# m1el/nemotron-asr.cpp

Hardware: AMD Instinct MI355X
Metric: RTFx (audio-sec/sec), nemotron-0.6B streaming forward path (higher is better)
Workload: dtype bf16

## Files before the change

nemotron-asr.cpp_amd/csrc/kernels_fused.hip:

```cpp
#include "nasr_internal.h"
#include "nasr_epilogue.h"
#include "nasr_wave.h"

namespace nasr {

typedef __attribute__((ext_vector_type(8))) __bf16 bf16x8;
typedef __attribute__((ext_vector_type(2))) __bf16 bf16x2;
typedef __attribute__((ext_vector_type(4))) float f32x4;
typedef __attribute__((ext_vector_type(4))) unsigned int u32x4;

__device__ __forceinline__ float wsum_f(float v) { return wave_sum(v); }
__device__ __forceinline__ float wmax_f(float v) { return wave_max(v); }

__device__ __forceinline__ int panel_byte(int row, int k, int KP) {
    const int chunk = k >> 3;
    return row * KP * 2 + (((chunk ^ (row & 15)) << 4) | ((k & 7) << 1));
}

__device__ __forceinline__ void store4_panel(char *panel, int row, int k, int KP, float a, float b, float c, float d) {
    uint2 r;
    r.x = (uint32_t)f32_to_bf16(a) | ((uint32_t)f32_to_bf16(b) << 16);
    r.y = (uint32_t)f32_to_bf16(c) | ((uint32_t)f32_to_bf16(d) << 16);
    *(uint2 *)(panel + panel_byte(row, k, KP)) = r;
}
// ... 1 lines not shown
__device__ __forceinline__ void wave_ln(float4 v[4], const float *w, const float *b, int lane) {
    float s = 0.f;
#pragma unroll
    for (int i = 0; i < 4; i++) s += (v[i].x + v[i].y) + (v[i].z + v[i].w);
    const float mean = wsum_f(s) * (1.0f / D);
    float q = 0.f;
#pragma unroll
    for (int i = 0; i < 4; i++) {
        v[i].x -= mean; v[i].y -= mean; v[i].z -= mean; v[i].w -= mean;
        q += (v[i].x * v[i].x + v[i].y * v[i].y) + (v[i].z * v[i].z + v[i].w * v[i].w);
    }
    const float inv = 1.0f / sqrtf(wsum_f(q) * (1.0f / D) + 1e-5f);
#pragma unroll
    for (int i = 0; i < 4; i++) {
        const int e = lane * 4 + 256 * i;
        const float4 ww = *(const float4 *)(w + e), bb = *(const float4 *)(b + e);
        v[i] = make_float4(v[i].x * inv * ww.x + bb.x, v[i].y * inv * ww.y + bb.y, v[i].z * inv * ww.z + bb.z, v[i].w * inv * ww.w + bb.w);
    }
}

__device__ __forceinline__ float bsum(float v, float *sh) {
    v = wsum_f(v);
    if ((threadIdx.x & 63) == 0) sh[threadIdx.x >> 6] = v;
    __syncthreads();
    return (sh[0] + sh[1]) + (sh[2] + sh[3]);
}
__device__ __forceinline__ float4 block_ln(float4 v, float4 ww, float4 bb, float *sh) {
    const float mean = bsum((v.x + v.y) + (v.z + v.w), sh) * (1.0f / D);
    const float dx = v.x - mean, dy = v.y - mean, dz = v.z - mean, dw = v.w - mean;
    const float var = bsum((dx * dx + dy * dy) + (dz * dz + dw * dw), sh + 4) * (1.0f / D);
    const float inv = 1.0f / sqrtf(var + 1e-5f);
    return make_float4(dx * inv * ww.x + bb.x, dy * inv * ww.y + bb.y, dz * inv * ww.z + bb.z, dw * inv * ww.w + bb.w);
}

template <bool BF16>
__device__ __forceinline__ float dot32(const float *qs, const void *row) {
    float s = 0.0f;
    if (BF16) {
        const uint4 *r = (const uint4 *)row;
#pragma unroll
        for (int c = 0; c < 4; c++) {
            const uint4 u = r[c];
            const uint32_t w[4] = {u.x, u.y, u.z, u.w};
#pragma unroll
            for (int e = 0; e < 4; e++) {
                s += qs[c * 8 + 2 * e] * __uint_as_float(w[e] << 16);
                s += qs[c * 8 + 2 * e + 1] * __uint_as_float(w[e] & 0xffff0000u);
            }
        }
    }
    return s;
}

#ifdef NASR_STAMPS
#define STAMP(i)                                                                                                         \
    do {                                                                                                                 \
        if (p.stamps && threadIdx.x == 0 && blockIdx.y == 0 && (blockIdx.x == 0 || blockIdx.x == gridDim.x - 1))          \
            p.stamps[(blockIdx.x == 0 ? 0 : 16) + (i)] = __builtin_amdgcn_s_memrealtime();                                \
    } while (0)
#else
#define STAMP(i)
#endif

#define PIN_SGPR(x) asm volatile("" ::"s"(x))

#ifndef GRP_OCC
#define GRP_OCC 4
#endif
template <int PRO, int MMAX>
__device__ __forceinline__ void fused_skinny_body(const FusedParams &p) {
    extern __shared__ __attribute__((aligned(16))) char smem[];
    const GemmParams &g = p.g;
    const int nt = blockIdx.x, split = blockIdx.y;
    const int wave = threadIdx.x >> 6, lane = threadIdx.x & 63;
    const int q = lane >> 4, r = lane & 15;
    const int KT = g.K >> 5;
    const int t0 = (int)((long)KT * split / g.splits), t1 = (int)((long)KT * (split + 1) / g.splits);
    const int KP = (t1 - t0) * 32;
    float *red = (float *)smem;
    char *panel = smem + 4096;
    const bool writer = blockIdx.x == 0 && blockIdx.y == 0;
    const int M = MMAX == 1 ? 1 : g.M;
    constexpr bool SMALL = MMAX <= 2;
    constexpr int MR = MMAX == 1 ? 1 : 2;
    STAMP(0);

    constexpr int U = (PRO == PRO_DWCONV && MMAX == 1) ? 2 : 8;
    const int nts = t1 - t0;
    const int w0 = t0 + nts * wave / 4, w1 = t0 + nts * (wave + 1) / 4;
    const u32x4 *wp = (const u32x4 *)g.W + (size_t)nt * KT * 64 + lane;
    u32x4 wv[U];
    auto issue_weights = [&]() {
        if (PRO == PRO_ATTN) {
#pragma unroll
            for (int u = 0; u < U; u++) {
                const int ntile = blockIdx.x * 8 + wave * 2 + (u >> 2), kt = t0 + (u & 3);
                wv[u] = __builtin_nontemporal_load((const u32x4 *)g.W + ((size_t)ntile * KT + kt) * 64 + lane);
            }
        } else {
#pragma unroll
            for (int u = 0; u < U; u++) {
                const int kt = w0 + u < w1 ? w0 + u : w1 - 1;
                wv[u] = __builtin_nontemporal_load(wp + (size_t)kt * 64);
            }
        }
        PIN_SGPR(g.epi); PIN_SGPR(g.out_f32); PIN_SGPR(g.ldo); PIN_SGPR(g.out_act); PIN_SGPR(g.ldo_act); PIN_SGPR(g.N);
        PIN_SGPR(g.q_out); PIN_SGPR(g.kv_pool); PIN_SGPR(g.kv_slot_stride); PIN_SGPR(g.rows); PIN_SGPR(g.T);
    };
    if (!((PRO == PRO_LN && SMALL) || PRO == PRO_ATTN || PRO == PRO_PLAIN || (PRO == PRO_DWCONV && SMALL))) issue_weights();
    STAMP(1);

    if (PRO == PRO_LN && SMALL) {
        const int c4 = threadIdx.x * 4;
        const float4 lw = *(const float4 *)(p.ln_w + c4), lb = *(const float4 *)(p.ln_b + c4);
        float4 ow = make_float4(0.f, 0.f, 0.f, 0.f), ob = ow;
        if (p.lno_w) { ow = *(const float4 *)(p.lno_w + c4); ob = *(const float4 *)(p.lno_b + c4); }
        float4 xv[MR], t[MR][8];
#pragma unroll
        for (int m = 0; m < MR; m++) {
            if (m < M) {
                xv[m] = *(const float4 *)(p.x_in + (size_t)m * D + c4);
#pragma unroll
                for (int sI = 0; sI < 8; sI++)
                    t[m][sI] = sI < p.part_splits ? *(const float4 *)(p.part + ((size_t)sI * M + m) * D + c4) : make_float4(0.f, 0.f, 0.f, 0.f);
            }
        }
        issue_weights();
#pragma unroll
        for (int m = 0; m < MR; m++) {
            if (m < M) {
                float4 v = xv[m];
                if (p.part_splits > 0) {
                    float4 o = t[m][0];
#pragma unroll
                    for (int sI = 1; sI < 8; sI++)
                        if (sI < p.part_splits) { o.x += t[m][sI].x; o.y += t[m][sI].y; o.z += t[m][sI].z; o.w += t[m][sI].w; }
                    v.x += p.scale * o.x; v.y += p.scale * o.y; v.z += p.scale * o.z; v.w += p.scale * o.w;
                }
                STAMP(2);
                if (p.lno_w) v = block_ln(v, ow, ob, red);
                if (writer && p.x_out) *(float4 *)(p.x_out + (size_t)m * D + c4) = v;
                v = block_ln(v, lw, lb, red);
                STAMP(3);
                store4_panel(panel, m, c4, KP, v.x, v.y, v.z, v.w);
            }
        }
        __syncthreads();
    } else if (PRO == PRO_LN) {
        float *xs = (float *)(panel + 16 * KP * 2);
        const int c4 = threadIdx.x * 4;
        for (int m0 = 0; m0 < M; m0 += 4) {
            float4 xv[4], t[4][8];
#pragma unroll
            for (int u = 0; u < 4; u++) {
                const int m = m0 + u < M ? m0 + u : M - 1;
                xv[u] = *(const float4 *)(p.x_in + (size_t)m * D + c4);
#pragma unroll
                for (int sI = 0; sI < 8; sI++)
                    t[u][sI] = sI < p.part_splits ? *(const float4 *)(p.part + ((size_t)sI * M + m) * D + c4) : make_float4(0.f, 0.f, 0.f, 0.f);
            }
#pragma unroll
            for (int u = 0; u < 4; u++) {
                const int m = m0 + u;
                if (m < M) {
                    float4 v = xv[u];
                    if (p.part_splits > 0) {
                        float4 o = t[u][0];
#pragma unroll
                        for (int sI = 1; sI < 8; sI++)
                            if (sI < p.part_splits) { o.x += t[u][sI].x; o.y += t[u][sI].y; o.z += t[u][sI].z; o.w += t[u][sI].w; }
                        v.x += p.scale * o.x; v.y += p.scale * o.y; v.z += p.scale * o.z; v.w += p.scale * o.w;
                    }
                    *(float4 *)(xs + (size_t)m * D + c4) = v;
                    if (writer && p.x_out && !p.lno_w) *(float4 *)(p.x_out + (size_t)m * D + c4) = v;
                }
            }
        }
        __syncthreads();
        for (int m = wave; m < M; m += 4) {
            float4 v[4];
#pragma unroll
            for (int i = 0; i < 4; i++) v[i] = *(const float4 *)(xs + (size_t)m * D + lane * 4 + 256 * i);
            if (p.lno_w) {
                wave_ln(v, p.lno_w, p.lno_b, lane);
                if (writer && p.x_out) {
#pragma unroll
                    for (int i = 0; i < 4; i++) *(float4 *)(p.x_out + (size_t)m * D + lane * 4 + 256 * i) = v[i];
                }
            }
            wave_ln(v, p.ln_w, p.ln_b, lane);
#pragma unroll
            for (int i = 0; i < 4; i++) store4_panel(panel, m, lane * 4 + 256 * i, KP, v[i].x, v[i].y, v[i].z, v[i].w);
        }
        __syncthreads();
    } else if (PRO == PRO_ATTN) {
        const AttnParams &a = p.at;
        const int h = split, T = a.T, KV = LCTX + T, TS = a.TS > 0 ? a.TS : a.T;
        float *qu = (float *)(panel + 16 * KP * 2);
        float *qv = qu + 16 * DH;
        float *sc = qv + 16 * DH;
        const int sub = threadIdx.x & 1;
        const int npair = M * KV;
        const float scale = 0.08838834764831845f;
        float qq = 0.f, bu = 0.f, bv = 0.f;
        if ((int)threadIdx.x < M * DH) {
            const int m = threadIdx.x >> 7, d = threadIdx.x & 127;
            qq = a.q[(size_t)m * D + h * DH + d]; bu = a.bias_u[h * DH + d]; bv = a.bias_v[h * DH + d];
        }
        RowDesc rds[2];
        rds[0] = a.rows[0];
        rds[1] = a.rows[(M - 1) / TS];
        auto pair_rows = [&](int pr, int &m, int &j, const bf16_t *&prow) {
            const bool ok = pr < npair;
            m = ok ? pr / KV : 0;
            j = ok ? pr - m * KV : 0;
            const int il = m - (m / TS) * TS, gch = il / T, i = il - gch * T;
            prow = (const bf16_t *)a.posproj + (size_t)(j + T - 1 - i) * D + h * DH + sub * 64;
            return ok;
        };
        auto key_row = [&](int m, int j) {
            const int b = m / TS, gch = (m - b * TS) / T;
            const RowDesc rd = b == 0 ? rds[0] : rds[1];
            int ring = rd.kv_head + gch * T + j;
            if (ring >= KVC) ring -= KVC;
            if (ring >= KVC) ring -= KVC;
            return (const bf16_t *)a.kv_pool + (size_t)rd.slot * a.kv_slot_stride + (size_t)ring * D + h * DH + sub * 64;
        };
        auto score = [&](const uint4 *kk, const uint4 *pp, int m, int j, bool ok) {
            const uint4 *qa = (const uint4 *)((const bf16_t *)qu + m * DH + sub * 64), *qb = (const uint4 *)((const bf16_t *)qv + m * DH + sub * 64);
            float s1 = 0.f, s2 = 0.f;
#pragma unroll
// ... 99 lines not shown
                    acc8[2 * e + 1] += w * __uint_as_float(vw[e] & 0xffff0000u);
                }
            }
            STAMP(6);
            float *pv = qu;
            *(float4 *)(pv + (wave * 4 + sr) * DH + c * 8) = make_float4(acc8[0], acc8[1], acc8[2], acc8[3]);
            *(float4 *)(pv + (wave * 4 + sr) * DH + c * 8 + 4) = make_float4(acc8[4], acc8[5], acc8[6], acc8[7]);
            __syncthreads();
            if ((int)threadIdx.x < DH) {
                const int d = threadIdx.x;
                float o = 0.f;
#pragma unroll
                for (int gI = 0; gI < 16; gI++) o += pv[gI * DH + d];
                *(bf16_t *)(panel + m * KP * 2 + ((((d >> 3) ^ (m & 15)) << 4) | ((d & 7) << 1))) = f32_to_bf16(o);
            }
            if (m + 1 < M) __syncthreads();
            }
        } else {
        int m0, j0;
        const bf16_t *prow0;
        const bool ok0 = pair_rows(threadIdx.x >> 1, m0, j0, prow0);
        uint4 kk[8], pp[8];
#pragma unroll
        for (int c = 0; c < 8; c++) pp[c] = ((const uint4 *)prow0)[c];
        issue_weights();
        const bf16_t *krow0 = key_row(m0, j0);
#pragma unroll
        for (int c = 0; c < 8; c++) kk[c] = ((const uint4 *)krow0)[c];
        uint2 vv[11];
        value_rows(0, vv);
        if ((int)threadIdx.x < M * DH) { ((bf16_t *)qu)[threadIdx.x] = f32_to_bf16(qq + bu); ((bf16_t *)qv)[threadIdx.x] = f32_to_bf16(qq + bv); }
        STAMP(2);
        __syncthreads();
        score(kk, pp, m0, j0, ok0);
        STAMP(3);
        if (MMAX > 1 && npair > 128) {
            int m1, j1;
            const bf16_t *prow1;
            const bool ok1 = pair_rows(128 + (threadIdx.x >> 1), m1, j1, prow1);
            const bf16_t *krow1 = key_row(m1, j1);
#pragma unroll
            for (int c = 0; c < 8; c++) { pp[c] = ((const uint4 *)prow1)[c]; kk[c] = ((const uint4 *)krow1)[c]; }
            score(kk, pp, m1, j1, ok1);
        }
        __syncthreads();
        for (int m = wave; m < M; m += 4) {
            const float v0 = lane < KV ? sc[m * KVC + lane] : -INFINITY;
            const float v1 = lane + 64 < KV ? sc[m * KVC + lane + 64] : -INFINITY;
            const float mx = wmax_f(fmaxf(v0, v1));
            const float e0 = lane < KV ? __expf(v0 - mx) : 0.0f;
            const float e1 = lane + 64 < KV ? __expf(v1 - mx) : 0.0f;
            const float inv = 1.0f / wsum_f(e0 + e1);
            if (lane < KV) sc[m * KVC + lane] = e0 * inv;
            if (lane + 64 < KV) sc[m * KVC + lane + 64] = e1 * inv;
        }
        __syncthreads();
        STAMP(6);
        {
            float *pv = qu;
            const int dq = threadIdx.x & 31, kgp = threadIdx.x >> 5;
            for (int m = 0; m < M; m++) {
                if (m > 0) value_rows(m, vv);
                float4 acc = make_float4(0.f, 0.f, 0.f, 0.f);
#pragma unroll
                for (int u = 0; u < 11; u++) {
                    const int jj = kgp + 8 * u;
                    const float w = jj < KV ? sc[m * KVC + jj] : 0.0f;
                    acc.x += w * __uint_as_float(vv[u].x << 16); acc.y += w * __uint_as_float(vv[u].x & 0xffff0000u);
                    acc.z += w * __uint_as_float(vv[u].y << 16); acc.w += w * __uint_as_float(vv[u].y & 0xffff0000u);
                }
                *(float4 *)(pv + (m * 8 + kgp) * DH + dq * 4) = acc;
            }
            __syncthreads();
            if ((int)threadIdx.x < M * DH) {
                const int m = threadIdx.x >> 7, d = threadIdx.x & 127;
                float o = 0.f;
#pragma unroll
                for (int gI = 0; gI < 8; gI++) o += pv[(m * 8 + gI) * DH + d];
                *(bf16_t *)(panel + m * KP * 2 + ((((d >> 3) ^ (m & 15)) << 4) | ((d & 7) << 1))) = f32_to_bf16(o);
            }
        }
        }
        __syncthreads();
    } else if (PRO == PRO_DWCONV) {
        const ConvParams &c = p.cv;
        const int T = c.T, ks1 = c.ks - 1;
        const int k0 = t0 * 32;
        if (SMALL) {
            const int c4 = threadIdx.x * 4;
            const float4 lw = *(const float4 *)(c.ln_w + c4), lb = *(const float4 *)(c.ln_b + c4);
            const RowDesc rd_first = c.rows[0];
            float4 w[9];
            if (c.ks == 9) {
#pragma unroll
                for (int k = 0; k < 9; k++) w[k] = *(const float4 *)(c.dw + (size_t)k * D + c4);
            }
            issue_weights();
            for (int m = 0; m < M; m++) {
                const int b = m / T, i = m - b * T;
                const RowDesc rd = b == 0 ? rd_first : c.rows[b];
                const float *cc_in = c.cc_pool + (size_t)rd.slot * c.cc_slot_stride + (size_t)rd.cc_par * ks1 * D;
                float *cc_out = c.cc_pool + (size_t)rd.slot * c.cc_slot_stride + (size_t)(rd.cc_par ^ 1) * ks1 * D;
                const float *gl = c.glu + (size_t)b * T * D;
                float4 acc;
                bool cache_written = false;
                if (c.ks == 9) {
                    float4 z[9];
#pragma unroll
                    for (int k = 0; k < 9; k++) {
                        const int rr = i + k;
                        z[k] = rr < 8 ? *(const float4 *)(cc_in + (size_t)rr * D + c4) : *(const float4 *)(gl + (size_t)(rr - 8) * D + c4);
                    }
                    acc = make_float4(z[0].x * w[0].x, z[0].y * w[0].y, z[0].z * w[0].z, z[0].w * w[0].w);
#pragma unroll
                    for (int k = 1; k < 9; k++) { acc.x += z[k].x * w[k].x; acc.y += z[k].y * w[k].y; acc.z += z[k].z * w[k].z; acc.w += z[k].w * w[k].w; }
                    if (writer && i == 0 && T == 1) {
#pragma unroll
                        for (int r2 = 0; r2 < 8; r2++) *(float4 *)(cc_out + (size_t)r2 * D + c4) = z[r2 + 1];
                        cache_written = true;
                    }
                } else {
                    acc = make_float4(0.f, 0.f, 0.f, 0.f);
                    for (int k = 0; k < c.ks; k++) {
                        const int rr = i + k;
                        const float4 z = rr < ks1 ? *(const float4 *)(cc_in + (size_t)rr * D + c4) : *(const float4 *)(gl + (size_t)(rr - ks1) * D + c4);
                        const float4 w = *(const float4 *)(c.dw + (size_t)k * D + c4);
                        if (k == 0) acc = make_float4(z.x * w.x, z.y * w.y, z.z * w.z, z.w * w.w);
                        else { acc.x += z.x * w.x; acc.y += z.y * w.y; acc.z += z.z * w.z; acc.w += z.w * w.w; }
                    }
                }
                float4 n = block_ln(acc, lw, lb, red);
                if (c4 >= k0 && c4 < k0 + KP) {
                    n.x = n.x / (1.0f + __expf(-n.x)); n.y = n.y / (1.0f + __expf(-n.y));
                    n.z = n.z / (1.0f + __expf(-n.z)); n.w = n.w / (1.0f + __expf(-n.w));
                    store4_panel(panel, m, c4 - k0, KP, n.x, n.y, n.z, n.w);
                }
                if (writer && i == 0 && !cache_written) {
                    for (int r2 = 0; r2 < ks1; r2++) {
                        const int rr = T + r2;
                        *(float4 *)(cc_out + (size_t)r2 * D + c4) =
                            rr < ks1 ? *(const float4 *)(cc_in + (size_t)rr * D + c4) : *(const float4 *)(gl + (size_t)(rr - ks1) * D + c4);
                    }
                }
            }
        } else {
            float *cs = (float *)(panel + 16 * KP * 2);
            const int c4 = threadIdx.x * 4;
            for (int m = 0; m < M; m++) {
                const int b = m / T, i = m - b * T;
                const RowDesc rd = c.rows[b];
                const float *cc_in = c.cc_pool + (size_t)rd.slot * c.cc_slot_stride + (size_t)rd.cc_par * ks1 * D;
                float *cc_out = c.cc_pool + (size_t)rd.slot * c.cc_slot_stride + (size_t)(rd.cc_par ^ 1) * ks1 * D;
                const float *gl = c.glu + (size_t)b * T * D;
                float4 acc;
                if (c.ks == 9) {
                    float4 z[9], w[9];
#pragma unroll
                    for (int k = 0; k < 9; k++) {
                        const int rr = i + k;
                        z[k] = rr < 8 ? *(const float4 *)(cc_in + (size_t)rr * D + c4) : *(const float4 *)(gl + (size_t)(rr - 8) * D + c4);
                        w[k] = *(const float4 *)(c.dw + (size_t)k * D + c4);
                    }
                    acc = make_float4(z[0].x * w[0].x, z[0].y * w[0].y, z[0].z * w[0].z, z[0].w * w[0].w);
#pragma unroll
                    for (int k = 1; k < 9; k++) { acc.x += z[k].x * w[k].x; acc.y += z[k].y * w[k].y; acc.z += z[k].z * w[k].z; acc.w += z[k].w * w[k].w; }
                } else {
                    acc = make_float4(0.f, 0.f, 0.f, 0.f);
                    for (int k = 0; k < c.ks; k++) {
                        const int rr = i + k;
                        const float4 z = rr < ks1 ? *(const float4 *)(cc_in + (size_t)rr * D + c4) : *(const float4 *)(gl + (size_t)(rr - ks1) * D + c4);
                        const float4 w = *(const float4 *)(c.dw + (size_t)k * D + c4);
                        if (k == 0) acc = make_float4(z.x * w.x, z.y * w.y, z.z * w.z, z.w * w.w);
                        else { acc.x += z.x * w.x; acc.y += z.y * w.y; acc.z += z.z * w.z; acc.w += z.w * w.w; }
                    }
                }
                *(float4 *)(cs + (size_t)m * D + c4) = acc;
                if (writer && i == 0) {
                    for (int r2 = 0; r2 < ks1; r2++) {
                        const int rr = T + r2;
                        *(float4 *)(cc_out + (size_t)r2 * D + c4) =
                            rr < ks1 ? *(const float4 *)(cc_in + (size_t)rr * D + c4) : *(const float4 *)(gl + (size_t)(rr - ks1) * D + c4);
                    }
                }
            }
            __syncthreads();
            for (int m = wave; m < M; m += 4) {
                float4 v[4];
#pragma unroll
                for (int ii = 0; ii < 4; ii++) v[ii] = *(const float4 *)(cs + (size_t)m * D + lane * 4 + 256 * ii);
                wave_ln(v, c.ln_w, c.ln_b, lane);
#pragma unroll
                for (int ii = 0; ii < 4; ii++) {
                    const int e = lane * 4 + 256 * ii;
                    if (e >= k0 && e < k0 + KP) {
                        float4 n = v[ii];
                        n.x = n.x / (1.0f + __expf(-n.x)); n.y = n.y / (1.0f + __expf(-n.y));
                        n.z = n.z / (1.0f + __expf(-n.z)); n.w = n.w / (1.0f + __expf(-n.w));
                        store4_panel(panel, m, e - k0, KP, n.x, n.y, n.z, n.w);
                    }
                }
            }
        }
        __syncthreads();
    }

    STAMP(4);
    uint4 avp[U];
    if (PRO == PRO_PLAIN) {
        const char *arow = (const char *)g.A + ((size_t)(r < M ? r : M - 1) * g.lda) * 2 + q * 16;
#pragma unroll
        for (int u = 0; u < U; u++) avp[u] = *(const uint4 *)(arow + (size_t)(w0 + u < w1 ? w0 + u : w1 - 1) * 64);
        issue_weights();
    }
    if (PRO == PRO_ATTN) {
        f32x4 a2[2] = {(f32x4){0.f, 0.f, 0.f, 0.f}, (f32x4){0.f, 0.f, 0.f, 0.f}};
#pragma unroll
        for (int u = 0; u < U; u++) {
            const uint4 av = *(const uint4 *)(panel + r * KP * 2 + (((((u & 3) << 2) | q) ^ r) << 4));
            a2[u >> 2] = __builtin_amdgcn_mfma_f32_16x16x32_bf16(__builtin_bit_cast(bf16x8, wv[u]), __builtin_bit_cast(bf16x8, av), a2[u >> 2], 0, 0, 0);
        }
        STAMP(5);
#pragma unroll
        for (int j = 0; j < 2; j++)
            epi_quad<true>(g, split, r, (blockIdx.x * 8 + wave * 2 + j) * 16 + q * 4, a2[j][0], a2[j][1], a2[j][2], a2[j][3]);
        STAMP(7);
        return;
    }
    f32x4 acc = (f32x4){0.f, 0.f, 0.f, 0.f};
#pragma unroll
    for (int u = 0; u < U; u++) {
        const int kt = w0 + u;
        if (kt < w1) {
            uint4 av;
            if (PRO == PRO_PLAIN) av = avp[u];
            else av = *(const uint4 *)(panel + r * KP * 2 + (((((kt - t0) << 2) | q) ^ r) << 4));
            acc = __builtin_amdgcn_mfma_f32_16x16x32_bf16(__builtin_bit_cast(bf16x8, wv[u]), __builtin_bit_cast(bf16x8, av), acc, 0, 0, 0);
        }
    }
    STAMP(5);
#pragma unroll
    for (int j = 0; j < 4; j++) red[(wave * 64 + lane) * 4 + j] = acc[j];
    __syncthreads();
    STAMP(6);
    if (wave == 0) {
        float v[4];
#pragma unroll
        for (int j = 0; j < 4; j++)
            v[j] = ((red[lane * 4 + j] + red[(64 + lane) * 4 + j]) + red[(128 + lane) * 4 + j]) + red[(192 + lane) * 4 + j];
        epi_quad<true>(g, split, r, nt * 16 + q * 4, v[0], v[1], v[2], v[3]);
    }
    STAMP(7);
}

template <int PRO, int MMAX>
__global__ __launch_bounds__(256, (MMAX == 1 && PRO != PRO_ATTN) ? 4 : 1) void k_fused_skinny(FusedParams p) {
    fused_skinny_body<PRO, MMAX>(p);
}
template <int PRO, int MMAX>
__global__ __launch_bounds__(256, (MMAX == 1 && PRO != PRO_ATTN) ? GRP_OCC : 1) void k_fused_skinny_grp(FusedParamsGroup pp) {
    const FusedParams &p = pp.p[blockIdx.z];
    if (p.g.M <= 0) return;
    fused_skinny_body<PRO, MMAX>(p);
}

void init_fused_kernel_attributes() {
    hipFuncSetAttribute((const void *)k_fused_skinny<PRO_LN, 16>, hipFuncAttributeMaxDynamicSharedMemorySize, 4096 + 32768 + 16 * D * 4);
    hipFuncSetAttribute((const void *)k_fused_skinny<PRO_DWCONV, 16>, hipFuncAttributeMaxDynamicSharedMemorySize, 4096 + 32768 + 16 * D * 4);
}

template <int MMAX>
static void launch_fused_m(const FusedParams &p, hipStream_t st, size_t lds) {
    const GemmParams &g = p.g;
    dim3 grid(g.N / 16, g.splits);
    switch (p.pro) {
    case PRO_LN: hipLaunchKernelGGL((k_fused_skinny<PRO_LN, MMAX>), grid, dim3(256), lds, st, p); break;
    case PRO_PLAIN: hipLaunchKernelGGL((k_fused_skinny<PRO_PLAIN, MMAX>), grid, dim3(256), 4096, st, p); break;
    case PRO_ATTN: hipLaunchKernelGGL((k_fused_skinny<PRO_ATTN, MMAX>), dim3(g.N / 128, g.splits), dim3(256), lds, st, p); break;
    case PRO_DWCONV: hipLaunchKernelGGL((k_fused_skinny<PRO_DWCONV, MMAX>), grid, dim3(256), lds, st, p); break;
    }
}

template <int MMAX>
static void launch_fused_grp_m(const FusedParamsGroup &pp, const FusedParams &p, int n, hipStream_t st, size_t lds) {
    const GemmParams &g = p.g;
    dim3 grid(g.N / 16, g.splits, n);
    switch (p.pro) {
    case PRO_LN: hipLaunchKernelGGL((k_fused_skinny_grp<PRO_LN, MMAX>), grid, dim3(256), lds, st, pp); break;
    case PRO_PLAIN: hipLaunchKernelGGL((k_fused_skinny_grp<PRO_PLAIN, MMAX>), grid, dim3(256), 4096, st, pp); break;
    case PRO_ATTN: hipLaunchKernelGGL((k_fused_skinny_grp<PRO_ATTN, MMAX>), dim3(g.N / 128, g.splits, n), dim3(256), lds, st, pp); break;
    case PRO_DWCONV: hipLaunchKernelGGL((k_fused_skinny_grp<PRO_DWCONV, MMAX>), grid, dim3(256), lds, st, pp); break;
    }
}

void launch_fused_skinny_group(const FusedParamsGroup &pp, int n, hipStream_t st) {
    int first = -1;
    for (int i = 0; i < n; i++)
        if (pp.p[i].g.M > 0) { first = i; break; }
    if (first < 0) return;
    const FusedParams &p = pp.p[first];
    const GemmParams &g = p.g;
    const int KP = (g.K / g.splits);
    size_t lds = 4096 + (size_t)16 * KP * 2;
    if (p.pro == PRO_ATTN) lds += (size_t)(2 * 16 * DH + 16 * KVC) * 4;
    const bool fits_u2 = p.pro != PRO_DWCONV || (g.K / 32 / g.splits + 3) / 4 <= 2;
    if (g.M == 1 && fits_u2) launch_fused_grp_m<1>(pp, p, n, st, lds);
    else launch_fused_grp_m<2>(pp, p, n, st, lds);
}

void launch_fused_skinny(const FusedParams &p, hipStream_t st) {
    const GemmParams &g = p.g;
    const int KP = (g.K / g.splits);
    size_t lds = 4096 + (size_t)16 * KP * 2;
    if (p.pro == PRO_ATTN) lds += (size_t)(2 * 16 * DH + 16 * KVC) * 4;
    if ((p.pro == PRO_LN || p.pro == PRO_DWCONV) && g.M > 2) lds += (size_t)g.M * D * 4;
    const bool fits_u2 = p.pro != PRO_DWCONV || (g.K / 32 / g.splits + 3) / 4 <= 2;
    if (g.M == 1 && fits_u2) launch_fused_m<1>(p, st, lds);
    else if (g.M <= 2) launch_fused_m<2>(p, st, lds);
    else launch_fused_m<16>(p, st, lds);
}

}
```

nemotron-asr.cpp_amd/csrc/nasr_encoder.hip:

```cpp
#include "nasr_engine_priv.h"

namespace nasr_eng {
double gemm_bytes(const nasr_engine *e, int M, int N, int K, int wesz) {
    return (double)N * K * wesz + (double)M * K * e->esz + (double)M * N * 4;
}

int run_gemm(nasr_engine *e, GemmParams &g, bool f32_weights, const char *tag) {
    (void)tag;
    const bool use_bf16 = e->bf16 && !f32_weights;
    const char *name = !use_bf16 ? "k_gemm_f32" : (g.M <= gemm_skinny_max_m() ? "k_gemm_skinny" : "k_gemm_tiled");
    ProfScope ps(e, name, gemm_bytes(e, g.M, g.N, g.K, use_bf16 ? 2 : 4), 2.0 * g.M * g.N * g.K);
    g.coresident = e->opt_gemm_cores == 0 ? 3 : e->opt_gemm_cores == 1 ? 2 : (e->gemm_coresident ? 1 : 0);
    g.f32_fma_tile = e->opt_f32_mfma ? 0 : 1;
    g.no_persist = e->opt_persist_gemm ? 0 : 1;
    g.no_wide = e->opt_wide_tiles ? 0 : 1;
    g.wide_rows = e->opt_wide_tiles == 256 ? 256 : e->opt_wide_tiles == 3 ? 2 : 0;
    g.tile_bands = e->opt_tile_bands < 0 ? 0 : e->opt_tile_bands == 0 ? 2 : 1;
    g.t64_tiles_p1 = e->opt_t64_tiles + 1;
    g.narrow_stores = e->opt_epilogue16 ? 0 : 1;
    g.prio = e->opt_gemm_prio;
    g.wide_min_tiles = e->opt_wide_min_tiles;
    g.wide_min_rows = e->opt_wide_min_rows;
    if (e->opt_ablate & 32) return 0;
    if (use_bf16) launch_gemm_bf16(g, e->st);
    else launch_gemm_f32(g, e->st);
    return 0;
}

int pick_splits(const nasr_engine *e, int M, int N, int K) {
    if (!e->bf16) return 1;
    const bool skinny = M <= gemm_skinny_max_m();
    int tasks = skinny ? (N / 16) * ((M + 63) / 64) : (N / gemm_tile_n(M, N, EPI_PART_F32, e->opt_t64_tiles + 1)) * ((M + 127) / 128);
    if (!skinny && (N / 128) * ((M + 127) / 128) >= (e->opt_split_tasks > 0 ? e->opt_split_tasks : 200)) return 1;
    if (!skinny) return tasks <= 40 ? 4 : (tasks < 256 ? 2 : 1);
    constexpr int skinny_cap = 8;
    int s = 1;
    while (s < skinny_cap && tasks * s < 256 && (K / 32) / (s * 2) >= 4) s *= 2;
    return s;
}

int run_layers_fused(nasr_engine *e, const RowDesc *rows, int B, int T, int G, int k0, int k1, std::vector<FusedParams> *rec) {
    const int TS = G * T;
    const int M = B * TS, nL = e->hp.n_layers, ks = e->hp.kernel_size;
    hipStream_t st = e->st;
    float *X[2] = {e->x, e->x2};
    int cur = 0;
    int prev_splits = 0;
    int kidx = 0;
#ifdef NASR_STAMPS
    unsigned long long *stamp_buf = g_stamp_buf + (size_t)g_stamp_pipe * STAMP_PER_SLOT * 32;
#endif
    auto launch = [&](FusedParams &f, const char *name, double bytes, double flops) {
        const int k = kidx++;
        if (k < k0 || k >= k1) return;
        if (rec) { rec->push_back(f); return; }
        ProfScope ps(e, name, bytes, flops);
#ifdef NASR_STAMPS
        f.stamps = stamp_buf + (size_t)k * 32;
#endif
        launch_fused_skinny(f, st);
    };
    auto wbytes = [&](int N, int K) { return (double)N * K * 2 + (double)M * (K + N) * 4; };
    for (int l = k0 / 8; l < (k1 + 7) / 8 && l < nL; l++) {
        LayerW &L = e->L[l];
        FusedParams f;
        kidx = 8 * l; cur = 0;
        prev_splits = l > 0 ? 4 : 0;
        memset(&f, 0, sizeof(f));
        f.pro = PRO_LN; f.x_in = X[cur]; f.x_out = X[cur ^ 1]; f.part = e->part; f.part_splits = prev_splits; f.scale = 0.5f;
        if (l > 0) { f.lno_w = e->L[l - 1].ln_out_w; f.lno_b = e->L[l - 1].ln_out_b; }
        f.ln_w = L.ln_ff1_w; f.ln_b = L.ln_ff1_b;
        f.g.W = L.ff1_w1; f.g.M = M; f.g.N = FF; f.g.K = D; f.g.splits = 1; f.g.epi = EPI_SILU_ACT; f.g.out_act = e->hbuf; f.g.ldo_act = FF;
        launch(f, "k_fused_ln_gemm", wbytes(FF, D), 2.0 * M * FF * D);
        cur ^= 1;
        memset(&f, 0, sizeof(f));
        f.pro = PRO_PLAIN; f.g.A = e->hbuf; f.g.lda = FF; f.g.W = L.ff1_w2; f.g.M = M; f.g.N = D; f.g.K = FF; f.g.splits = 4;
        f.g.epi = EPI_PART_F32; f.g.out_f32 = e->part; f.g.ldo = D;
        launch(f, "k_fused_plain_gemm", wbytes(D, FF), 2.0 * M * D * FF);
        memset(&f, 0, sizeof(f));
        f.pro = PRO_LN; f.x_in = X[cur]; f.x_out = X[cur ^ 1]; f.part = e->part; f.part_splits = 4; f.scale = 0.5f;
        f.ln_w = L.ln_att_w; f.ln_b = L.ln_att_b;
        f.g.W = L.wqkv; f.g.M = M; f.g.N = 3 * D; f.g.K = D; f.g.splits = 1; f.g.epi = EPI_QKV; f.g.q_out = e->q;
        f.g.kv_pool = e->kv_pool[l]; f.g.kv_slot_stride = (int64_t)2 * KVC * D; f.g.rows = rows; f.g.T = TS;
        launch(f, "k_fused_ln_gemm", wbytes(3 * D, D), 2.0 * M * 3 * D * D);
        cur ^= 1;
        constexpr int fuse_max_m = FUSE_MAX_M;
        int wo_splits = NH;
        if (M <= fuse_max_m) {
            memset(&f, 0, sizeof(f));
            f.pro = PRO_ATTN; f.at.q = e->q; f.at.kv_pool = e->kv_pool[l]; f.at.kv_slot_stride = (int64_t)2 * KVC * D; f.at.act_bf16 = 1;
            f.at.posproj = L.posproj[T]; f.at.bias_u = L.bias_u; f.at.bias_v = L.bias_v; f.at.rows = rows; f.at.B = B; f.at.T = T; f.at.TS = TS;
            f.g.W = L.wo; f.g.M = M; f.g.N = D; f.g.K = D; f.g.splits = NH; f.g.epi = EPI_PART_F32; f.g.out_f32 = e->part; f.g.ldo = D;
            launch(f, "k_fused_attn_gemm", wbytes(D, D) + (double)B * (3.0 * (LCTX + T)) * D * 2, 2.0 * M * D * D);
        } else {
            AttnParams ap;
            memset(&ap, 0, sizeof(ap));
            ap.q = e->q; ap.kv_pool = e->kv_pool[l]; ap.kv_slot_stride = (int64_t)2 * KVC * D; ap.act_bf16 = 1;
            ap.posproj = L.posproj[T]; ap.bias_u = L.bias_u; ap.bias_v = L.bias_v; ap.rows = rows; ap.B = B; ap.T = T; ap.TS = TS;
            ap.ctx_out = e->ctx;
            if (kidx >= k0 && kidx < k1) { ProfScope ps(e, "k_attention", (double)B * (3.0 * (LCTX + T)) * D * 2, 2.0 * M * (LCTX + T) * D * 3); launch_attention(ap, st); }
            wo_splits = 4;
            memset(&f, 0, sizeof(f));
            f.pro = PRO_PLAIN; f.g.A = e->ctx; f.g.lda = D; f.g.W = L.wo; f.g.M = M; f.g.N = D; f.g.K = D; f.g.splits = 4;
            f.g.epi = EPI_PART_F32; f.g.out_f32 = e->part; f.g.ldo = D;
            launch(f, "k_fused_plain_gemm", wbytes(D, D), 2.0 * M * D * D);
        }
        memset(&f, 0, sizeof(f));
        f.pro = PRO_LN; f.x_in = X[cur]; f.x_out = X[cur ^ 1]; f.part = e->part; f.part_splits = wo_splits; f.scale = 1.0f;
        f.ln_w = L.ln_conv_w; f.ln_b = L.ln_conv_b;
        f.g.W = L.pw1; f.g.M = M; f.g.N = 2 * D; f.g.K = D; f.g.splits = 1; f.g.epi = EPI_GLU; f.g.out_f32 = e->glu; f.g.ldo = D;
        launch(f, "k_fused_ln_gemm", wbytes(2 * D, D), 2.0 * M * 2 * D * D);
        cur ^= 1;
        const int pw2_splits = 4;
        if (M <= fuse_max_m) {
            memset(&f, 0, sizeof(f));
            f.pro = PRO_DWCONV; f.cv.glu = e->glu; f.cv.cc_pool = e->cc_pool[l]; f.cv.cc_slot_stride = (int64_t)2 * (ks - 1) * D;
            f.cv.dw = L.dw; f.cv.ln_w = L.cln_w; f.cv.ln_b = L.cln_b; f.cv.rows = rows; f.cv.B = B; f.cv.T = TS; f.cv.ks = ks;
            f.g.W = L.pw2; f.g.M = M; f.g.N = D; f.g.K = D; f.g.splits = pw2_splits; f.g.epi = EPI_PART_F32; f.g.out_f32 = e->part; f.g.ldo = D;
            launch(f, "k_fused_dwconv_gemm", wbytes(D, D), 2.0 * M * D * D);
        } else {
            ConvParams cp;
            memset(&cp, 0, sizeof(cp));
            cp.glu = e->glu; cp.cc_pool = e->cc_pool[l]; cp.cc_slot_stride = (int64_t)2 * (ks - 1) * D;
            cp.dw = L.dw; cp.ln_w = L.cln_w; cp.ln_b = L.cln_b; cp.rows = rows; cp.B = B; cp.T = TS; cp.ks = ks;
            cp.c_out = e->cbuf; cp.act_bf16 = 1;
            if (kidx >= k0 && kidx < k1) { ProfScope ps(e, "k_dwconv", (double)M * D * 6 + (double)B * 2 * (ks - 1) * D * 4, 2.0 * M * D * ks); launch_dwconv(cp, st); }
            memset(&f, 0, sizeof(f));
            f.pro = PRO_PLAIN; f.g.A = e->cbuf; f.g.lda = D; f.g.W = L.pw2; f.g.M = M; f.g.N = D; f.g.K = D; f.g.splits = 4;
            f.g.epi = EPI_PART_F32; f.g.out_f32 = e->part; f.g.ldo = D;
            launch(f, "k_fused_plain_gemm", wbytes(D, D), 2.0 * M * D * D);
        }
        memset(&f, 0, sizeof(f));
        f.pro = PRO_LN; f.x_in = X[cur]; f.x_out = X[cur ^ 1]; f.part = e->part; f.part_splits = pw2_splits; f.scale = 1.0f;
        f.ln_w = L.ln_ff2_w; f.ln_b = L.ln_ff2_b;
        f.g.W = L.ff2_w1; f.g.M = M; f.g.N = FF; f.g.K = D; f.g.splits = 1; f.g.epi = EPI_SILU_ACT; f.g.out_act = e->hbuf; f.g.ldo_act = FF;
        launch(f, "k_fused_ln_gemm", wbytes(FF, D), 2.0 * M * FF * D);
        cur ^= 1;
        memset(&f, 0, sizeof(f));
        f.pro = PRO_PLAIN; f.g.A = e->hbuf; f.g.lda = FF; f.g.W = L.ff2_w2; f.g.M = M; f.g.N = D; f.g.K = FF; f.g.splits = 4;
        f.g.epi = EPI_PART_F32; f.g.out_f32 = e->part; f.g.ldo = D;
        launch(f, "k_fused_plain_gemm", wbytes(D, FF), 2.0 * M * D * FF);
        prev_splits = 4;
    }
    if (k1 < 8 * nL || rec) return 0;
    cur = 0;
    PostParams q;
    memset(&q, 0, sizeof(q));
    q.x = X[cur]; q.M = M; q.part = e->part; q.splits = 4; q.scale = 0.5f; q.ln_out = 1;
    q.ln1_w = e->L[nL - 1].ln_out_w; q.ln1_b = e->L[nL - 1].ln_out_b;
    if (X[cur] != e->x) q.copy_out = e->x;
    ProfScope ps(e, "k_post", (double)M * D * 24);
    launch_post(q, st);
    return 0;
}

int enqueue_encoder(nasr_engine *e, const RowDesc *rows, const RowDesc *vrows, const int *tap_slots, int B, int T, int R, int G, int seg,
                           int nseg, int part) {
    const int Bs = B * G;
    const int M = Bs * T;
    const int chunk_mel = PRE_CACHE + 8 * (1 + R);
    hipStream_t st = e->st;
    const int act = e->bf16 ? 1 : 0;
    const int nLayers = e->hp.n_layers;
    const int shift = nseg == 2 && nLayers >= 8 ? 1 : 0;
    auto bound = [&](int k) {
        if (k <= 0) return 0;
        if (k >= nseg) return nLayers;
        if (nseg == 3 && nLayers >= 6) return k == 1 ? nLayers * 7 / 24 : nLayers * 16 / 24;
        if (nseg == 4 && nLayers >= 8) return k == 1 ? nLayers * 6 / 24 : k == 2 ? nLayers * 13 / 24 : nLayers * 20 / 24;
        return std::max(1, nLayers * k / nseg - shift);
    };
    const int l0 = bound(seg), l1 = bound(seg + 1);
    const bool front = part == 0 ? seg == 0 : part == 1, tail = part == 0 ? seg == nseg - 1 : part == 2;
    GemmParams g;

    auto tap_copy = [&](float *tap_base, size_t per_slot, size_t layer_off) -> int {
        for (int b = 0; b < B; b++)
            HIPCHK(hipMemcpyAsync(tap_base + (size_t)tap_slots[b] * per_slot + layer_off, e->x + (size_t)b * T * D,
                                  (size_t)T * D * 4, hipMemcpyDeviceToDevice, st));
        return 0;
    };
    const int H1 = chunk_mel / 2 + 1, W1 = 65, H2 = H1 / 2 + 1, W2 = 33, H3 = H2 / 2 + 1, W3 = 17;
    if (front && !(e->opt_ablate & 16)) {
    {
        ProfScope ps(e, "k_sub_conv0_dw", (double)Bs * (chunk_mel * NMEL * 4 + H2 * W2 * SUBC * (act ? 2 : 4)), 2.0 * Bs * H2 * W2 * SUBC * 90);
        launch_sub_conv0_dw(vrows, Bs, chunk_mel, e->mel_ring, e->w0t, e->b0, e->w2t, e->b2, e->sub_b, act, H1, W1, st);
    }
    memset(&g, 0, sizeof(g));
    g.A = e->sub_b; g.W = e->w3; g.M = Bs * H2 * W2; g.N = SUBC; g.K = SUBC; g.lda = SUBC; g.splits = 1;
    g.epi = EPI_BIAS_RELU_F32; g.out_f32 = e->sub_a; g.ldo = SUBC; g.bias = e->b3;
    run_gemm(e, g, false, "sub_pw3");
    {
        ProfScope ps(e, "k_sub_dw", (double)B * H2 * W2 * SUBC * 4, 2.0 * B * H3 * W3 * SUBC * 9);
        launch_sub_dw(e->sub_a, Bs, H2, W2, e->w5t, e->b5, e->sub_b, act, st);
    }
    memset(&g, 0, sizeof(g));
    g.A = e->sub_b; g.W = e->w6; g.M = Bs * H3 * W3; g.N = SUBC; g.K = SUBC; g.lda = SUBC; g.splits = 1;
// ... 325 lines not shown
```

nemotron-asr.cpp_amd/csrc/nasr_internal.h:

```cpp
#pragma once
#include <hip/hip_runtime.h>
#include <stdint.h>

namespace nasr {

constexpr int D      = 1024;
constexpr int NH     = 8;
constexpr int DH     = 128;
constexpr int FF     = 4096;
constexpr int NMEL   = 128;
constexpr int NBINS  = 257;
constexpr int NFFT   = 512;
constexpr int HOP    = 160;
constexpr int WIN    = 400;
constexpr int LCTX   = 70;
constexpr int TMAX   = 14;
constexpr int MAXNEW = 256;
constexpr int KVC    = LCTX + MAXNEW;
constexpr int SUBC   = 256;
constexpr int SUBF   = 17;
constexpr int SUBFLAT = SUBC * SUBF;
constexpr int VOCAB  = 1025;
constexpr int BLANK  = 1024;
constexpr int HID    = 640;
// ... 120 lines not shown
void launch_gemm_f32(const GemmParams &p, hipStream_t st);
void launch_pack_weight_bf16(const float *w_f32, bf16_t *packed, int N, int K, hipStream_t st);
void launch_f32_to_bf16(const float *in, bf16_t *out, int64_t n, hipStream_t st);

struct MelParams {
    const PcmDesc *desc; int B; int max_frames;
    float *abuf;
    float *last_sample;
    float *mel_ring;
    const float *window;
    const float *fbT;
    const int *fb_band;
    const float *cos_t, *sin_t;
    float *tap; int tap_cap;
};
void launch_mel(const MelParams &p, int max_n, hipStream_t st);
void launch_mel_put(const float *staged, const PcmDesc *desc, int B, int max_frames, float *mel_ring, hipStream_t st);
void launch_mel_zero(const PcmDesc *desc, int B, int max_frames, float *mel_ring, hipStream_t st);
struct StreamResetParams {
    float *const *cc_pools;
    void *const *kv_pools;
    int esz, kv_head;
    int n_layers, slot;
    int cc_slot_floats;
    int keep_reference_state;
    float *abuf, *last_sample, *mel_ring, *dec_h, *dec_c;
    DecCtrl *ctrl;
};
void launch_stream_reset(const StreamResetParams &p, hipStream_t st);

void launch_sub_conv0_dw(const RowDesc *rows, int B, int chunk_mel, const float *mel_ring, const float *w0t, const float *b0,
                         const float *w2t, const float *b2, void *out, int out_bf16, int H1, int W1, hipStream_t st);
void launch_sub_dw(const float *in, int B, int Hin, int Win, const float *wt, const float *bias, void *out,
                   int out_bf16, hipStream_t st);

void launch_post(const PostParams &p, hipStream_t st);

struct AttnParams {
    const float *q;
    const void *kv_pool; int64_t kv_slot_stride; int act_bf16;
    const void *posproj;
    const float *bias_u, *bias_v;
    const RowDesc *rows; int B; int T;
    int TS;
    void *ctx_out;
    int ablate;
};
void launch_attention(const AttnParams &p, hipStream_t st);

struct ConvParams {
    const float *glu;
    float *cc_pool; int64_t cc_slot_stride;
    const float *dw;
    const float *ln_w, *ln_b;
    const RowDesc *rows; int B; int T; int ks;
    void *c_out; int act_bf16;
    int stream_form;
};
void launch_dwconv(const ConvParams &p, hipStream_t st);

struct DecParams {
    const RowDesc *rows; int B; int T;
    DecCtrl *ctrl;
    float *h, *c;
    const float *encproj;
    const float *embed;
    const float *w_ih[2], *w_hh[2], *b_ih[2], *b_hh[2];
    const float *pred_w, *pred_b, *out_w, *out_b;
    float *predg;
    unsigned long long *key;
    int *n_active;
    int *n_dirty;
    int *n_rows;
    int *dlist;
    unsigned *rowmap;
    int *tok_ring;
    int *tok_frame;
};
void launch_decode_begin(const DecParams &p, hipStream_t st);
void launch_decode_iter(const DecParams &p, int iter, hipStream_t st);
int decode_blind_iterations(int frames);
void launch_encproj(const float *x, const float *wpk, const float *bias, float *out, int M, int K, int N, hipStream_t st);

enum Pro { PRO_LN = 0, PRO_PLAIN = 1, PRO_ATTN = 2, PRO_DWCONV = 3 };
struct FusedParams {
    GemmParams g;
    int pro;
    const float *x_in; float *x_out; const float *part; int part_splits; float scale;
    const float *lno_w, *lno_b;
    const float *ln_w, *ln_b;
    AttnParams at;
    ConvParams cv;
#ifdef NASR_STAMPS
    unsigned long long *stamps;
#endif
};
void launch_fused_skinny(const FusedParams &p, hipStream_t st);
constexpr int FUSED_GROUP = 4;
struct FusedParamsGroup { FusedParams p[FUSED_GROUP]; };
void launch_fused_skinny_group(const FusedParamsGroup &pp, int n, hipStream_t st);

void launch_prompt_add_relu(float *h, const float *w1p, const RowDesc *rows, int M, int T, int P, hipStream_t st);
void launch_relu(float *x, int64_t n, hipStream_t st);
void launch_fill_f32(float *p, float v, int64_t n, hipStream_t st);

__device__ __forceinline__ float bf16_to_f32(bf16_t v) {
    return __uint_as_float(((uint32_t)v) << 16);
}
__device__ __forceinline__ bf16_t f32_to_bf16(float f) {
    uint32_t u = __float_as_uint(f);
    if ((u & 0x7fffffffu) > 0x7f800000u) return (bf16_t)((u >> 16) | 0x40);
    return (bf16_t)((u + 0x7fffu + ((u >> 16) & 1u)) >> 16);
}


constexpr int DIAR_NMEL = 80;
constexpr int VAD_WINDOW = 10080, VAD_T = 64, VAD_TVALID = 63;
constexpr int SPK_SEGMENT = 24000, SPK_T = 160, SPK_TVALID = 150;
constexpr int SPK_EMB = 192, SPK_C = 3072, SPK_ATT = 128;

struct DiarMelParams {
    const float *audio;
    const int16_t *audio_s16;
    const long long *win_off;
    int n_win;
    int T_pad, t_valid;
    int cpitch;
    float *mel;
    const float *window;
    const float *fbT;
    const int *fb_band;
    const float *cos_t, *sin_t;
};
void launch_diar_logmel(const DiarMelParams &p, int W, bool per_feature_normalize, hipStream_t st);
struct DiarFrameDesc { long long base; int n; int t; };
void launch_diar_frames(const DiarMelParams &p, const DiarFrameDesc *frames, int n_frames, float *out, hipStream_t st);

struct VadSub { const float *dw, *pw, *scale, *bias; int kernel, dil, cin, cout; const bf16_t *pw16; };
struct VadNet {
    VadSub sub[9];
    VadSub res[3];
    const float *dec_w, *dec_b;
};
void launch_vad_marblenet(const VadNet &net, const float *shared, const float *edge, const int *win_row, const int *lens_mel,
                          float *prob, int W, hipStream_t st);
void launch_vad_marblenet_bf16(const VadNet &net, const float *shared, const float *edge, const int *win_row, const int *lens_mel,
                               float *prob, int W, hipStream_t st);
void launch_vad_marblenet_f16(const VadNet &net, const float *shared, const float *edge, const int *win_row, const int *lens_mel,
                              float *prob, int W, hipStream_t st);
void init_diar_kernel_attributes();

enum { SG_DW = 0, SG_Y = 1, SG_RES = 2, SG_ASP = 3 };
struct SpkGemmParams {
    const bf16_t *A; int lda;
    const bf16_t *W;
    int S, N, K, mode;
    const float *bias;
    const int *lens;
    const float *dw_w; int dw_k;
    bf16_t *a_out; int lda_out;
    float *y_out, *colmean;
    const float *y_in, *z;
    bf16_t *x_out;
    const bf16_t *x_in;
    const float *bn_s, *bn_b; float *pool;
#ifdef SG_STAMPS
    unsigned long long *stamps;
// ... 40 lines not shown
```

Baseline: 188.2.

## Fold depthwise conv into pw1 GLU epilogue and LN+SiLU into pw2 prologue

For small M with kernel size 9, the depthwise convolution moves into the epilogue of the LN+pw1 GEMM. The GLU output is combined with the cached conv context and neighbouring rows, which are fetched through lane shuffles. The pw2 GEMM then gets a lighter prologue that only applies the conv LayerNorm and SiLU. This shortens the serial work and global traffic in the pw2 prologue. The cost is extra register pressure and context loads in the pw1 epilogue, and two new template instantiations.

Result: no change. 189.1, median of 6 (+0.5%).

```diff
diff --git a/nemotron-asr.cpp_amd/csrc/kernels_fused.hip b/nemotron-asr.cpp_amd/csrc/kernels_fused.hip
--- a/nemotron-asr.cpp_amd/csrc/kernels_fused.hip
+++ b/nemotron-asr.cpp_amd/csrc/kernels_fused.hip
@@ -107,10 +107,12 @@
     const bool writer = blockIdx.x == 0 && blockIdx.y == 0;
     const int M = MMAX == 1 ? 1 : g.M;
     constexpr bool SMALL = MMAX <= 2;
+    constexpr bool LNP = PRO == PRO_LN || PRO == PRO_LN_DWCONV;
+    static_assert((PRO != PRO_LN_DWCONV && PRO != PRO_CONVLN) || SMALL, "the conv-in-pw1 forms exist for M <= 2 only");
     constexpr int MR = MMAX == 1 ? 1 : 2;
     STAMP(0);
 
-    constexpr int U = (PRO == PRO_DWCONV && MMAX == 1) ? 2 : 8;
+    constexpr int U = ((PRO == PRO_DWCONV || PRO == PRO_CONVLN) && MMAX == 1) ? 2 : 8;
     const int nts = t1 - t0;
     const int w0 = t0 + nts * wave / 4, w1 = t0 + nts * (wave + 1) / 4;
     const u32x4 *wp = (const u32x4 *)g.W + (size_t)nt * KT * 64 + lane;
@@ -132,10 +134,13 @@
         PIN_SGPR(g.epi); PIN_SGPR(g.out_f32); PIN_SGPR(g.ldo); PIN_SGPR(g.out_act); PIN_SGPR(g.ldo_act); PIN_SGPR(g.N);
         PIN_SGPR(g.q_out); PIN_SGPR(g.kv_pool); PIN_SGPR(g.kv_slot_stride); PIN_SGPR(g.rows); PIN_SGPR(g.T);
     };
-    if (!((PRO == PRO_LN && SMALL) || PRO == PRO_ATTN || PRO == PRO_PLAIN || (PRO == PRO_DWCONV && SMALL))) issue_weights();
+    if (!((LNP && SMALL) || PRO == PRO_ATTN || PRO == PRO_PLAIN || ((PRO == PRO_DWCONV || PRO == PRO_CONVLN) && SMALL))) issue_weights();
     STAMP(1);
 
-    if (PRO == PRO_LN && SMALL) {
+    RowDesc crd0, crd1;
+    if (PRO == PRO_LN_DWCONV) { crd0 = p.cv.rows[0]; crd1 = p.cv.rows[(M - 1) / p.cv.T]; }
+
+    if (LNP && SMALL) {
         const int c4 = threadIdx.x * 4;
         const float4 lw = *(const float4 *)(p.ln_w + c4), lb = *(const float4 *)(p.ln_b + c4);
         float4 ow = make_float4(0.f, 0.f, 0.f, 0.f), ob = ow;
@@ -151,6 +156,9 @@
             }
         }
         issue_weights();
+        if (PRO == PRO_LN_DWCONV) {
+            PIN_SGPR(crd0.slot); PIN_SGPR(crd0.cc_par); PIN_SGPR(crd1.slot); PIN_SGPR(crd1.cc_par);
+        }
 #pragma unroll
         for (int m = 0; m < MR; m++) {
             if (m < M) {
@@ -171,7 +179,7 @@
             }
         }
         __syncthreads();
-    } else if (PRO == PRO_LN) {
+    } else if (LNP) {
         float *xs = (float *)(panel + 16 * KP * 2);
         const int c4 = threadIdx.x * 4;
         for (int m0 = 0; m0 < M; m0 += 4) {
@@ -437,6 +445,28 @@
         }
         }
         __syncthreads();
+    } else if (PRO == PRO_CONVLN) {
+        const ConvParams &c = p.cv;
+        const int k0 = t0 * 32;
+        const int c4 = threadIdx.x * 4;
+        const float4 lw = *(const float4 *)(c.ln_w + c4), lb = *(const float4 *)(c.ln_b + c4);
+        float4 xv[MR];
+#pragma unroll
+        for (int m = 0; m < MR; m++)
+            if (m < M) xv[m] = *(const float4 *)(c.glu + (size_t)m * D + c4);
+        issue_weights();
+#pragma unroll
+        for (int m = 0; m < MR; m++) {
+            if (m < M) {
+                float4 n = block_ln(xv[m], lw, lb, red);
+                if (c4 >= k0 && c4 < k0 + KP) {
+                    n.x = n.x / (1.0f + __expf(-n.x)); n.y = n.y / (1.0f + __expf(-n.y));
+                    n.z = n.z / (1.0f + __expf(-n.z)); n.w = n.w / (1.0f + __expf(-n.w));
+                    store4_panel(panel, m, c4 - k0, KP, n.x, n.y, n.z, n.w);
+                }
+            }
+        }
+        __syncthreads();
     } else if (PRO == PRO_DWCONV) {
         const ConvParams &c = p.cv;
         const int T = c.T, ks1 = c.ks - 1;
@@ -560,6 +590,17 @@
     }
 
     STAMP(4);
+    float2 cz[8], cw[9];
+    if (PRO == PRO_LN_DWCONV) {
+        const ConvParams &c = p.cv;
+        const int mr = r < M ? r : M - 1, b = mr / c.T, i = mr - b * c.T;
+        const int slot = b == 0 ? crd0.slot : crd1.slot, par = b == 0 ? crd0.cc_par : crd1.cc_par;
+        const float *cc_in = c.cc_pool + (size_t)slot * c.cc_slot_stride + (size_t)par * 8 * D + nt * 8 + q * 2;
+#pragma unroll
+        for (int k = 0; k < 8; k++) cz[k] = *(const float2 *)(cc_in + (size_t)(i + k < 8 ? i + k : 7) * D);
+#pragma unroll
+        for (int k = 0; k < 9; k++) cw[k] = *(const float2 *)(c.dw + (size_t)k * D + nt * 8 + q * 2);
+    }
     uint4 avp[U];
     if (PRO == PRO_PLAIN) {
         const char *arow = (const char *)g.A + ((size_t)(r < M ? r : M - 1) * g.lda) * 2 + q * 16;
@@ -602,7 +643,36 @@
 #pragma unroll
         for (int j = 0; j < 4; j++)
             v[j] = ((red[lane * 4 + j] + red[(64 + lane) * 4 + j]) + red[(128 + lane) * 4 + j]) + red[(192 + lane) * 4 + j];
-        epi_quad<true>(g, split, r, nt * 16 + q * 4, v[0], v[1], v[2], v[3]);
+        if (PRO == PRO_LN_DWCONV) {
+            const ConvParams &c = p.cv;
+            const int ch = nt * 8 + q * 2;
+            const float2 gl = make_float2(v[0] * sigmoid_f(v[1]), v[2] * sigmoid_f(v[3]));
+            const int mr = r < M ? r : M - 1, b = mr / c.T, i = mr - b * c.T;
+            float2 z[9];
+#pragma unroll
+            for (int k = 0; k < 8; k++) z[k] = cz[k];
+            z[8] = gl;
+#pragma unroll
+            for (int k = 9 - MMAX; k < 8; k++) {
+                const int src = i + k >= 8 ? lane + k - 8 : lane;
+                const float gx = __shfl(gl.x, src), gy = __shfl(gl.y, src);
+                if (i + k >= 8) z[k] = make_float2(gx, gy);
+            }
+            float2 acc = make_float2(z[0].x * cw[0].x, z[0].y * cw[0].y);
+#pragma unroll
+            for (int k = 1; k < 9; k++) { acc.x += z[k].x * cw[k].x; acc.y += z[k].y * cw[k].y; }
+            if (r < M) {
+                *(float2 *)(g.out_f32 + (size_t)r * g.ldo + ch) = acc;
+                if (i == c.T - 1) {
+                    const int slot = b == 0 ? crd0.slot : crd1.slot, par = b == 0 ? crd0.cc_par : crd1.cc_par;
+                    float *cc_out = c.cc_pool + (size_t)slot * c.cc_slot_stride + (size_t)(par ^ 1) * 8 * D + ch;
+#pragma unroll
+                    for (int r2 = 0; r2 < 8; r2++) *(float2 *)(cc_out + (size_t)r2 * D) = z[r2 + 1];
+                }
+            }
+        } else {
+            epi_quad<true>(g, split, r, nt * 16 + q * 4, v[0], v[1], v[2], v[3]);
+        }
     }
     STAMP(7);
 }
@@ -632,6 +702,8 @@
     case PRO_PLAIN: hipLaunchKernelGGL((k_fused_skinny<PRO_PLAIN, MMAX>), grid, dim3(256), 4096, st, p); break;
     case PRO_ATTN: hipLaunchKernelGGL((k_fused_skinny<PRO_ATTN, MMAX>), dim3(g.N / 128, g.splits), dim3(256), lds, st, p); break;
     case PRO_DWCONV: hipLaunchKernelGGL((k_fused_skinny<PRO_DWCONV, MMAX>), grid, dim3(256), lds, st, p); break;
+    case PRO_LN_DWCONV: if constexpr (MMAX <= 2) hipLaunchKernelGGL((k_fused_skinny<PRO_LN_DWCONV, MMAX>), grid, dim3(256), lds, st, p); break;
+    case PRO_CONVLN: if constexpr (MMAX <= 2) hipLaunchKernelGGL((k_fused_skinny<PRO_CONVLN, MMAX>), grid, dim3(256), lds, st, p); break;
     }
 }
 
@@ -644,6 +716,8 @@
     case PRO_PLAIN: hipLaunchKernelGGL((k_fused_skinny_grp<PRO_PLAIN, MMAX>), grid, dim3(256), 4096, st, pp); break;
     case PRO_ATTN: hipLaunchKernelGGL((k_fused_skinny_grp<PRO_ATTN, MMAX>), dim3(g.N / 128, g.splits, n), dim3(256), lds, st, pp); break;
     case PRO_DWCONV: hipLaunchKernelGGL((k_fused_skinny_grp<PRO_DWCONV, MMAX>), grid, dim3(256), lds, st, pp); break;
+    case PRO_LN_DWCONV: hipLaunchKernelGGL((k_fused_skinny_grp<PRO_LN_DWCONV, MMAX>), grid, dim3(256), lds, st, pp); break;
+    case PRO_CONVLN: hipLaunchKernelGGL((k_fused_skinny_grp<PRO_CONVLN, MMAX>), grid, dim3(256), lds, st, pp); break;
     }
 }
 
@@ -657,7 +731,7 @@
     const int KP = (g.K / g.splits);
     size_t lds = 4096 + (size_t)16 * KP * 2;
     if (p.pro == PRO_ATTN) lds += (size_t)(2 * 16 * DH + 16 * KVC) * 4;
-    const bool fits_u2 = p.pro != PRO_DWCONV || (g.K / 32 / g.splits + 3) / 4 <= 2;
+    const bool fits_u2 = (p.pro != PRO_DWCONV && p.pro != PRO_CONVLN) || (g.K / 32 / g.splits + 3) / 4 <= 2;
     if (g.M == 1 && fits_u2) launch_fused_grp_m<1>(pp, p, n, st, lds);
     else launch_fused_grp_m<2>(pp, p, n, st, lds);
 }
@@ -668,7 +742,8 @@
     size_t lds = 4096 + (size_t)16 * KP * 2;
     if (p.pro == PRO_ATTN) lds += (size_t)(2 * 16 * DH + 16 * KVC) * 4;
     if ((p.pro == PRO_LN || p.pro == PRO_DWCONV) && g.M > 2) lds += (size_t)g.M * D * 4;
-    const bool fits_u2 = p.pro != PRO_DWCONV || (g.K / 32 / g.splits + 3) / 4 <= 2;
+    const bool fits_u2 = (p.pro != PRO_DWCONV && p.pro != PRO_CONVLN) || (g.K / 32 / g.splits + 3) / 4 <= 2;
+    if ((p.pro == PRO_LN_DWCONV || p.pro == PRO_CONVLN) && (g.M > 2 || !fits_u2)) return;
     if (g.M == 1 && fits_u2) launch_fused_m<1>(p, st, lds);
     else if (g.M <= 2) launch_fused_m<2>(p, st, lds);
     else launch_fused_m<16>(p, st, lds);
diff --git a/nemotron-asr.cpp_amd/csrc/nasr_encoder.hip b/nemotron-asr.cpp_amd/csrc/nasr_encoder.hip
--- a/nemotron-asr.cpp_amd/csrc/nasr_encoder.hip
+++ b/nemotron-asr.cpp_amd/csrc/nasr_encoder.hip
@@ -105,14 +105,25 @@
             f.g.epi = EPI_PART_F32; f.g.out_f32 = e->part; f.g.ldo = D;
             launch(f, "k_fused_plain_gemm", wbytes(D, D), 2.0 * M * D * D);
         }
+        const bool conv_in_pw1 = M <= fuse_max_m && ks == 9;
         memset(&f, 0, sizeof(f));
-        f.pro = PRO_LN; f.x_in = X[cur]; f.x_out = X[cur ^ 1]; f.part = e->part; f.part_splits = wo_splits; f.scale = 1.0f;
+        f.pro = conv_in_pw1 ? PRO_LN_DWCONV : PRO_LN; f.x_in = X[cur]; f.x_out = X[cur ^ 1]; f.part = e->part; f.part_splits = wo_splits; f.scale = 1.0f;
         f.ln_w = L.ln_conv_w; f.ln_b = L.ln_conv_b;
         f.g.W = L.pw1; f.g.M = M; f.g.N = 2 * D; f.g.K = D; f.g.splits = 1; f.g.epi = EPI_GLU; f.g.out_f32 = e->glu; f.g.ldo = D;
-        launch(f, "k_fused_ln_gemm", wbytes(2 * D, D), 2.0 * M * 2 * D * D);
+        if (conv_in_pw1) {
+            f.cv.cc_pool = e->cc_pool[l]; f.cv.cc_slot_stride = (int64_t)2 * (ks - 1) * D; f.cv.dw = L.dw;
+            f.cv.rows = rows; f.cv.B = B; f.cv.T = TS; f.cv.ks = ks;
+        }
+        launch(f, conv_in_pw1 ? "k_fused_ln_gemm_dwconv" : "k_fused_ln_gemm",
+               wbytes(2 * D, D) + (conv_in_pw1 ? (double)B * 2 * (ks - 1) * D * 4 + (double)ks * D * 4 : 0.0), 2.0 * M * 2 * D * D);
         cur ^= 1;
         const int pw2_splits = 4;
-        if (M <= fuse_max_m) {
+        if (conv_in_pw1) {
+            memset(&f, 0, sizeof(f));
+            f.pro = PRO_CONVLN; f.cv.glu = e->glu; f.cv.ln_w = L.cln_w; f.cv.ln_b = L.cln_b; f.cv.B = B; f.cv.T = TS; f.cv.ks = ks;
+            f.g.W = L.pw2; f.g.M = M; f.g.N = D; f.g.K = D; f.g.splits = pw2_splits; f.g.epi = EPI_PART_F32; f.g.out_f32 = e->part; f.g.ldo = D;
+            launch(f, "k_fused_convln_gemm", wbytes(D, D), 2.0 * M * D * D);
+        } else if (M <= fuse_max_m) {
             memset(&f, 0, sizeof(f));
             f.pro = PRO_DWCONV; f.cv.glu = e->glu; f.cv.cc_pool = e->cc_pool[l]; f.cv.cc_slot_stride = (int64_t)2 * (ks - 1) * D;
             f.cv.dw = L.dw; f.cv.ln_w = L.cln_w; f.cv.ln_b = L.cln_b; f.cv.rows = rows; f.cv.B = B; f.cv.T = TS; f.cv.ks = ks;
diff --git a/nemotron-asr.cpp_amd/csrc/nasr_internal.h b/nemotron-asr.cpp_amd/csrc/nasr_internal.h
--- a/nemotron-asr.cpp_amd/csrc/nasr_internal.h
+++ b/nemotron-asr.cpp_amd/csrc/nasr_internal.h
@@ -226,7 +226,7 @@
 int decode_blind_iterations(int frames);
 void launch_encproj(const float *x, const float *wpk, const float *bias, float *out, int M, int K, int N, hipStream_t st);
 
-enum Pro { PRO_LN = 0, PRO_PLAIN = 1, PRO_ATTN = 2, PRO_DWCONV = 3 };
+enum Pro { PRO_LN = 0, PRO_PLAIN = 1, PRO_ATTN = 2, PRO_DWCONV = 3, PRO_LN_DWCONV = 4, PRO_CONVLN = 5 };
 struct FusedParams {
     GemmParams g;
     int pro;
```
